# yeyupiaoling/PPASR

Hardware: AMD Instinct MI355X
Metric: audio-seconds/s (RTF^-1) Conformer-streaming fbank, batch32 per GPU, ctc_greedy (higher is better)
Workload: dtype f32; 1 GPU; configs[1]: Conformer streaming (configs/conformer.yml), fbank-80, 32 x 10 s utterances per GPU, V=4233, ctc_greedy, features resident in HBM -> token ids + scores on device; global_batch=32, frames=1000, decoder=ctc_greedy, parallelism=utterance-dp1, pipelined=False, gemm=f32

## Files before the change

### ppasr_amd/csrc/capi.hip

```cpp
#include <cstdlib>

#include "capi_internal.h"

namespace ppasr {
thread_local LaunchProf g_launch_prof;
}

static thread_local std::string g_err;
std::string& ppasr_err_slot() { return g_err; }

static ppasr_status validate_desc(const ppasr_model_desc* desc, ppasr_model_s* m) {
  m->desc = *desc;
  const int F = desc->input_dim;
  if (desc->model_type == PPASR_MODEL_DEEPSPEECH2) {
    if (F > 128 || F < 7) return fail(PPASR_EUNSUPPORTED, "input_dim out of range");
    m->F1 = (F - 1) / 2;
    m->F2 = (m->F1 - 1) / 2;
    if (m->F1 > 40) return fail(PPASR_EUNSUPPORTED, "deepspeech2: input_dim <= 82 ((input_dim - 1) / 2 <= 40)");
    return PPASR_OK;
  }
  if (desc->model_type != PPASR_MODEL_CONFORMER && desc->model_type != PPASR_MODEL_SQUEEZEFORMER &&
      desc->model_type != PPASR_MODEL_EFFICIENT_CONFORMER)
    return fail(PPASR_EUNSUPPORTED, "model_type not built (conformer, efficient_conformer, squeezeformer are)");
  const bool eff = desc->model_type == PPASR_MODEL_EFFICIENT_CONFORMER;
// ... 30 lines not shown
    return fail(PPASR_EINVAL, "PPASR_OPT_SQ_NO_ADAPTIVE_SCALE / PPASR_OPT_SQ_PRE_NORM are Squeezeformer options");
  if (desc->linear_units % 256 != 0 || desc->linear_units <= 0) return fail(PPASR_EUNSUPPORTED, "linear_units % 256 != 0");
  if (!generic && !fused_ks) return fail(PPASR_EUNSUPPORTED, "cnn_module_kernel must be 7, 15 or 31");
  if (generic) {
    const int ks = desc->cnn_module_kernel;
    const bool use_cnn = !(desc->options & PPASR_OPT_NO_CNN);
    if (use_cnn && (ks < 1 || ks > 63 || (!desc->causal && ks % 2 == 0)))
      return fail(PPASR_EINVAL, "cnn_module_kernel: 1..63, odd for the non-causal conv module (convolution.py:38)");
    if ((desc->options & PPASR_OPT_POS_MASK) == 3 || ((desc->options >> PPASR_OPT_ACT_SHIFT) & PPASR_OPT_ACT_MASK) > PPASR_ACT_HARDSHRINK)
      return fail(PPASR_EINVAL, "options: unknown pos_enc_layer_type / activation_type code");
  }
  if (desc->model_type == PPASR_MODEL_SQUEEZEFORMER && desc->cnn_module_kernel == 7)
    return fail(PPASR_EUNSUPPORTED, "squeezeformer: cnn_module_kernel must be 15 or 31");
  if (desc->input_dim > 128 || (desc->input_dim < 7 && desc->input_layer != 1) || desc->input_dim < 1)
    return fail(PPASR_EUNSUPPORTED, "input_dim out of range");
  if (eff) {
    m->desc.stride_layer_mask = (int)smask;
    m->desc.stride_layer_idx = smask ? __builtin_ctz(smask) : -1;
  }
  const int il = desc->input_layer;
  if (il != 0 && il != 1 && il != 6 && il != 8)
    return fail(PPASR_EINVAL, "input_layer: 0 (conv2d), 1 (linear), 6 (conv2d6) or 8 (conv2d8)");
  m->generic = generic;
  m->gen.pos = desc->options & PPASR_OPT_POS_MASK;
  m->gen.post_norm = (desc->options & PPASR_OPT_POST_NORM) != 0;
  m->gen.concat_after = (desc->options & PPASR_OPT_CONCAT_AFTER) != 0;
  m->gen.macaron = !(desc->options & PPASR_OPT_NO_MACARON);
  m->gen.use_cnn = !(desc->options & PPASR_OPT_NO_CNN);
  m->gen.act = (desc->options >> PPASR_OPT_ACT_SHIFT) & PPASR_OPT_ACT_MASK;
  m->gen.sq_pre_norm = (desc->options & PPASR_OPT_SQ_PRE_NORM) != 0;
  if (il != 0 && desc->model_type == PPASR_MODEL_SQUEEZEFORMER)
    return fail(PPASR_EUNSUPPORTED, "squeezeformer: only the conv2d front end is built");
  m->F1 = (F - 1) / 2;
  if (il == 6 && m->F1 < 5) return fail(PPASR_EINVAL, "input_dim too small for this input_layer (conv2d6: >= 11)");
  m->F2 = il == 6 ? (m->F1 - 5) / 3 + 1 : (m->F1 - 1) / 2;
  m->F3 = il == 8 ? (m->F2 - 1) / 2 : 0;
  if (il != 1 && m->F_last() < 1) return fail(PPASR_EINVAL, "input_dim too small for this input_layer");
  return PPASR_OK;
}

extern "C" {

const char* ppasr_last_error(void) { return g_err.c_str(); }
const char* ppasr_version(void) { return "ppasr_hip 0.1 (gfx950, fp32 MFMA)"; }

ppasr_status ppasr_create(const ppasr_model_desc* desc, const ppasr_weight_blob* blobs, int n_blobs, ppasr_handle* out) {
  if (!desc || !blobs || !out) return fail(PPASR_EINVAL, "null argument");
  std::unique_ptr<ppasr_model_s> m(new ppasr_model_s());
  LOAD_TRY(validate_desc(desc, m.get()));
  HIP_TRY(configure_kernels());
  if (desc->model_type != PPASR_MODEL_DEEPSPEECH2) {
    HIP_TRY(configure_generic_kernels());
    HIP_TRY(configure_squeezeformer_kernels());
  }
  const BlobMap sd = blob_map(blobs, n_blobs);
  Loader ld{m.get(), sd, ""};
  switch (desc->model_type) {
    case PPASR_MODEL_DEEPSPEECH2: LOAD_TRY(ds2_create(m.get(), ld)); break;
    case PPASR_MODEL_SQUEEZEFORMER: LOAD_TRY(squeezeformer_create(m.get(), ld)); break;
    default: LOAD_TRY(conformer_create(m.get(), ld));
  }
  HIP_TRY(hipDeviceSynchronize());
  *out = m.release();
  return PPASR_OK;
}

ppasr_status ppasr_destroy(ppasr_handle h) {
  delete h;
  return PPASR_OK;
}

int ppasr_out_frames(ppasr_handle h, int T) {
  if (T < (h ? h->min_frames() : 7)) return 0;
  int tp = h ? h->front_dims(T).Tp : ((T - 1) / 2 - 1) / 2;
  if (h)
    for (int n = __builtin_popcount(eff_stride_mask(h->desc)); n > 0; --n) tp = (tp + 1) / 2;
  return tp;
}

}
WsLayout ws_layout(const ppasr_model_s* m, int B, int T) {
  if (m->generic) {
    WsLayout g{};
    g.total = generic_ws_floats(m, B, T);
    return g;
  }
  const auto fd = m->front_dims(T);
  const size_t T1 = fd.T1, Tp = fd.Tp;
  const size_t M = (size_t)B * Tp;
  auto al = [](size_t n) { return (n + 63) & ~(size_t)63; };
  WsLayout w;
  size_t o = 0;
  const size_t split_rows = m->ffn_split > 1 ? (size_t)m->ffn_split * M
                          : m->ffn_split == 0 ? 0 : std::min((size_t)8 * M, (size_t)256 * kRows);
  w.y1 = o; o += al(std::max((size_t)B * T1 * m->F1 * kD, 4 * split_rows * kD));
  const size_t y2_floats = (size_t)B * (fd.T2 ? fd.T2 : Tp) * m->F2 * kD;
  w.y2 = o; o += al(m->desc.input_layer == 8 ? std::max(y2_floats, split_rows * kD) : y2_floats);
  w.xa = o; o += al(M * kD);
  w.xb = o; o += al(M * kD);
  w.xc = o; o += al(M * kD);
  w.qkv = o; o += al(M * 3 * kD);
  w.ctx = o; o += al(M * kD);
  w.g = o; o += al(M * kD);
  w.rmax = o; o += al(M);
  w.rsum = o; o += al(M);
  w.fa = o; o += al(M);
// ... 463 lines not shown
```

### ppasr_amd/csrc/capi_internal.h

```cpp
#pragma once
#include <hip/hip_runtime.h>

#include <cmath>
#include <cstdio>
#include <cstring>
#include <memory>
#include <string>
#include <unordered_map>
#include <vector>

#include "../../include/ppasr_hip.h"
#include "conformer_kernels.h"
#include "launch.h"
#include "ctc_beam.h"

using namespace ppasr;

#include "squeezeformer_kernels.h"
#include "ds2_kernels.h"
#include "rescore_kernels.h"

std::string& ppasr_err_slot();
inline ppasr_status fail(ppasr_status s, const std::string& msg) {
  ppasr_err_slot() = msg;
// ... 138 lines not shown
  };
  int sub_rate() const { return desc.input_layer == 1 ? 1 : desc.input_layer ? desc.input_layer : 4; }
  int F_last() const { return desc.input_layer == 8 ? F3 : F2; }
  int min_frames() const { return desc.input_layer == 1 ? 1 : desc.input_layer == 6 ? 11 : desc.input_layer == 8 ? 15 : 7; }
  Front front_dims(int T) const {
    if (desc.input_layer == 1) return Front{0, 0, T};
    Front f{(T - 1) / 2, 0, 0};
    if (desc.input_layer == 6) {
      f.Tp = (f.T1 - 5) / 3 + 1;
    } else if (desc.input_layer == 8) {
      f.T2 = (f.T1 - 1) / 2;
      f.Tp = (f.T2 - 1) / 2;
    } else {
      f.Tp = (f.T1 - 1) / 2;
    }
    return f;
  }
  bool generic = false;
  struct GenOpts {
    int pos = 0;
    bool post_norm = false, concat_after = false, macaron = true, use_cnn = true;
    int act = 0;
    bool sq_pre_norm = false;
  } gen;
  struct GenLayerX {
    const f32x4* wcat = nullptr;
    const float* bcat = nullptr;
  };
  std::vector<GenLayerX> gen_x;
  const float* pe_dev = nullptr;
  const float* zero_vec = nullptr;
  const float *lin_ln_g = nullptr, *lin_ln_b = nullptr;
  int lin_kpad = 0;
  FrontW front;
  std::vector<LayerW> layers;
  std::vector<int> layer_ks;
  std::vector<int> layer_group;
  HeadW head;
  std::vector<SqLayerW> sq_layers;
  SqReduceW sq_reduce{};
  const f32x4* sq_wrec = nullptr;
  const float* sq_brec = nullptr;
  const float *preln_g = nullptr, *preln_b = nullptr;
  Ds2W ds2{};
  int ds2_persist_hold = 0, ds2_persist_giveups = 0;
  std::vector<Ds2LayerW> ds2_layers;
  float* taps = nullptr;
  size_t taps_floats = 0;
  float* memory_out = nullptr;
  size_t memory_floats = 0;
  bool sq_final_proj = false;
  bool prof = false;
  int front_fused = -1;
  int ffn_split = -1;
  bool skip_padding = false;
  int gemm_mode = 0;
  std::vector<LayerW> layers_h3;
  const f32x4* conv2_w_h3 = nullptr;
  const f32x4* embed_w_h3 = nullptr;
  const f32x4* head_w_h3 = nullptr;
  std::vector<SqLayerW> sq_layers_h3;
  bool h3_layers() const { return gemm_mode == PPASR_GEMM_F16X3 && !layers_h3.empty(); }
  bool h3_sq_layers() const { return gemm_mode == PPASR_GEMM_F16X3 && !sq_layers_h3.empty(); }
  int gemm_coverage = 0;
  bool gemm_guard = true;
  static constexpr int kGuardN = 5;
  unsigned int* guard_ctr[kGuardN] = {};
  unsigned int* guard_dev = nullptr;
  unsigned int* guard_host = nullptr;
  unsigned int guard_seen[kGuardN] = {};
  long long guard_fallbacks = 0, guard_events = 0;
  int row_block = -1;
  std::vector<int64_t> lens_hint;
  std::vector<hipEvent_t> ev_pool;
  size_t ev_used = 0;
  struct Span { int cls; std::vector<std::pair<hipEvent_t, hipEvent_t>> ev; };
  std::vector<Span> spans;

  ppasr_status upload(const std::vector<float>& v, const float** out) {
    return upload_bytes(v.data(), v.size() * sizeof(float), reinterpret_cast<const void**>(out));
  }
  ppasr_status upload4(const std::vector<float>& v, const f32x4** out) {
    return upload_bytes(v.data(), v.size() * sizeof(float), reinterpret_cast<const void**>(out));
  }
  hipEvent_t next_event() {
    if (ev_used == ev_pool.size()) {
      hipEvent_t e;
      (void)hipEventCreate(&e);
      ev_pool.push_back(e);
    }
    return ev_pool[ev_used++];
  }
  ~ppasr_model_s() {
    for (hipEvent_t e : ev_pool) (void)hipEventDestroy(e);
    if (guard_host) (void)hipHostFree(guard_host);
  }
};


struct ppasr_stream_s {
  ppasr_model_s* m;
  int D;
  int cap;
  int cache_t;
  int cache_r;
  int offset;
// ... 58 lines not shown
```

### ppasr_amd/csrc/conformer_kernels.h

```cpp
#pragma once
#include <hip/hip_runtime.h>
#include <stdint.h>

#include "rowblock.h"

namespace ppasr {

struct LayerW {
  const float *ln_mac_g, *ln_mac_b, *ln_mha_g, *ln_mha_b, *ln_conv_g, *ln_conv_b;
  const float *ln_ff_g, *ln_ff_b, *ln_fin_g, *ln_fin_b, *ln_cm_g, *ln_cm_b;
  float cm_eps;
  const f32x4 *ffm_w1, *ffm_w2, *ff_w1, *ff_w2, *wqkv, *wo, *pw1, *pw2;
  const float *ffm_b1, *ffm_b2, *ff_b1, *ff_b2, *bqkv, *bo, *pw1_b, *pw2_b;
  const float *dw_w;
  const float *dw_b;
  const float *glu_pad;
  const float *pos_u, *pos_v;
  const float *ptab;
  const float *dtab = nullptr;
};

struct FrontW {
  const float *cmvn_mean, *cmvn_istd;
  const float *conv1_w, *conv1_b;
// ... 17 lines not shown
struct SessDesc {
  int sess;
  int cache_t;
  int pos0;
  int offset;
};

struct AttnArgs {
  const float* q;
  int q_stride;
  const float* k;
  int k_stride;
  const float* v;
  int v_stride;
  int T1, T2;
  int pos0;
  const int64_t* lens;
  float* ctx;
  const float *pos_u, *pos_v;
  const float* ptab;
  int pos_stride;
  int mask_mul;
  int q_frames, kv_frames;
  int group;
  const SessDesc* sess;
  long long sess_stride;
  int pad_skip;
  const float* vt = nullptr;
  int vt_stride = 0;
  int dm = 256;
  const float* dtab = nullptr;
  int dtab_len = 0;
};
struct VtOut {
  float* vt = nullptr;
  int stride = 0;
  int k_h3 = 0;
  const float* kpos = nullptr;
  int kpos_stride = 0;
  int Ti = 1;
};

constexpr size_t kLdsExclusive = 82 * 1024;
size_t ragged_lds(size_t lds, const PadSkip& ps, int n_blocks);

bool launch_attention_t(const AttnArgs& a, int B, int H, hipStream_t st);
hipError_t configure_attention_kernels();

void launch_block_table(const PadSkip& ps, int M, int R, int* tab, hipStream_t st);

bool conv2_quad_supported(const FrontW& fw);
bool conv12_supported(const FrontW& fw, int F, int F2);
void launch_conv12(const float* feats, const FrontW& fw, float* y2, int B, int T, int F, int Tp, int F2, hipStream_t st,
                   const PadSkip& ps_frames, int* tile_scratch);
void launch_conv2_quad(const float* y1, const FrontW& fw, float* y2, int B, int T1, int F1, int Tp, int F2, hipStream_t st,
                       const PadSkip& ps_frames, int* tile_scratch);
hipError_t configure_front_fused_kernels();

void launch_out_glu_split_16(const float* ctx, const float* x1, float* x2, float* g, float* xhat, const LayerW& w,
                             const int64_t* lens, int M, int Tp, int mask_mul, hipStream_t st, const PadSkip& ps,
                             float* hist = nullptr, int lo = 0);
void launch_shift_caches(float* kc, float* vc, long long layer_stride, int D, int n_layers, int from_full, int keep_full,
                         int from_half, int keep_half, unsigned long long half_mask, hipStream_t st);
void launch_oproj_ln_16(const float* ctx, const float* x1, float* x2_sink, float* xhat_out, const LayerW& w, int M,
                        hipStream_t st, const PadSkip& ps = PadSkip{});
void launch_pw1_glu_cols_16(const float* x, float* g, const LayerW& w, int M, hipStream_t st, float* hist = nullptr, int lo = 0,
                            const float* hist_scale = nullptr, const float* hist_bias = nullptr, const PadSkip& ps = PadSkip{},
                            const int64_t* lens = nullptr, int Tp = 1, int mask_mul = 1);
bool conv_ffn_16_supported(int ksize, int Tp);
hipError_t configure_conformer_t_kernels();

template <int R>
struct LayerStagesT {
  static hipError_t configure();
  static void ffn_qkv(const float* x_in, float* x1, float* qkv, const LayerW& w, int M, int n_chunks, hipStream_t st,
                      const PadSkip& ps, VtOut vt);
  static void out_glu(const float* ctx, const float* x1, float* x2, float* g, const LayerW& w, const int64_t* lens, int M,
                      int Tp, int mask_mul, hipStream_t st, const PadSkip& ps, float* xhat_out = nullptr,
                      int stop_after_ln = 0);
  static void conv_ffn(const float* g, const float* x2, float* x_out, const LayerW& w, const int64_t* lens, int M, int Tp,
                       int n_chunks, int ksize, int mask_mul, const LayerW* next, float* x1_next, float* qkv_next,
                       hipStream_t st, bool causal, const PadSkip& ps, VtOut vt_next);
};

void launch_posproj(const float* pe, const float* wpos , const float* bpos_or_null, float* ptab,
                    int max_len, hipStream_t st, int d = 256);
void launch_pos_dtab(const float* ptab, const float* pos_u, const float* pos_v, float* dtab, int max_len, hipStream_t st);
void launch_conv1(const float* feats, const FrontW& fw, float* y1, int B, int T, int F, int T1, int F1, hipStream_t st,
                  const PadSkip& ps = PadSkip{}, int channels = 256);
void launch_conv_stage(const float* y_in, const f32x4* w, const float* bias, float* y_out, int B, int T_in, int F_in,
                       int T_out, int F_out, int k, int s, hipStream_t st, const PadSkip& ps_frames = PadSkip{},
                       int channels = 256, int* tile_scratch = nullptr,
                       bool h3 = false,
                       float* part = nullptr, size_t part_floats = 0);
size_t conv_stage_part_floats(int M, int channels = 256);
size_t conv_stage_part_reserve(int M);
void launch_conv2(const float* y1, const FrontW& fw, float* y2, int B, int T1, int F1, int Tp, int F2, hipStream_t st,
                  const PadSkip& ps = PadSkip{}, int* tile_scratch = nullptr, const f32x4* w_h3 = nullptr, float* part = nullptr,
                  size_t part_floats = 0);
void launch_embed(const float* y2, const FrontW& fw, float* x0, int M, int K, float xscale, bool scale_before_bias,
                  hipStream_t st, const PadSkip& ps = PadSkip{}, int k_slices = 1, float* part = nullptr,
                  const f32x4* w_h3 = nullptr);
void launch_dense(const float* a, int lda, const f32x4* w, const float* bias, float* out, int M, int K, int n_cols_padded,
                  int ldc, int n_valid, hipStream_t st, float scale = 1.0f, float* part = nullptr, size_t part_floats = 0);
void launch_ffn_qkv(const float* x_in, float* x1, float* qkv, const LayerW& w, int M, int n_chunks, hipStream_t st,
                    const PadSkip& ps = PadSkip{}, VtOut vt = VtOut{}, bool h3 = false, int rows = 32);
void launch_repack_h3(const f32x4* src, f32x4* dst, int n_tiles, int G, unsigned int* ovf, hipStream_t st);
inline bool conv_ffn_h3_supported(int ksize) { return ksize == 15 || ksize == 7; }
void launch_split_rows_h3(const float* src, float* dst, long long n_rows, unsigned int* ovf, hipStream_t st);
// ... 88 lines not shown
```

### ppasr_amd/csrc/encode_common.h

```cpp
#pragma once

struct RaggedPlan {
  bool skip;
  const int64_t* lens;
  int rc;
  bool rate_changes;
  int mul0;
  int slack(int mul) const { return rate_changes && mul == mul0 ? 2 * (rc + 4) + rc + 8 : rc + 4; }
  PadSkip at(int Tcur, int mul) const {
    PadSkip ps;
    if (skip) {
      ps.lens = lens;
      ps.Tp = Tcur;
      ps.mul = mul;
      ps.slack = slack(mul);
    }
    return ps;
  }
  int attn_pad_skip(const PadSkip& ps) const { return skip ? ps.slack + 1 : 0; }
};

struct BlockTables {
  struct Tab { int Ti, R; int* tab; } tabs[4];
  int n = 0, B;
// ... 5 lines not shown
      : B(B_), off(((size_t)B_ + 2 + 15) / 16 * 16), cap(2 * (((size_t)M + 63) / 64 * 64)), base(reinterpret_cast<int*>(stats)), st(st_) {
    fits = (size_t)B + 2 <= cap / 2;
    on = skip && fits && block_tables_enabled();
  }
  int* tile_tab() const { return fits ? base : nullptr; }
  PadSkip make(PadSkip p, int Tcur, int R) {
    const size_t len = 1 + ((size_t)B * Tcur + R - 1) / R;
    if (!on || n == 4 || off + len > cap) return p;
    int* t = base + off;
    launch_block_table(p, B * Tcur, R, t, st);
    tabs[n++] = Tab{Tcur, R, t};
    off += (len + 15) / 16 * 16;
    p.tab = t;
    return p;
  }
  PadSkip with_table(PadSkip p, int Tcur, int R) {
    for (int k = 0; k < n; ++k)
      if (tabs[k].Ti == Tcur && tabs[k].R == R) {
        p.tab = tabs[k].tab;
        return p;
      }
    return make(p, Tcur, R);
  }
};

struct Taps {
  float* buf;
  size_t cap;
  hipStream_t st;
  size_t off = 0;
  void operator()(const float* src, size_t n_floats) {
    if (buf && off + n_floats <= cap)
      (void)hipMemcpyAsync(buf + off, src, n_floats * sizeof(float), hipMemcpyDeviceToDevice, st);
    off += n_floats;
  }
};

struct NoSpans {
  template <typename Fn>
  void operator()(int, Fn&& fn) const { fn(); }
};

template <typename Spans>
inline void front4_fused(const ppasr_model_s* h, const float* feats, int B, int T, const PadSkip& ps, int* tile_tab,
                         bool scale_before_bias, int embed_slices, const PadSkip& ps_embed, float* y1, float* y2, float* xa,
                         hipStream_t st, Spans&& spans) {
  const auto fd = h->front_dims(T);
  const int F = h->desc.input_dim, T1 = fd.T1, F1 = h->F1, Tp = fd.Tp, F2 = h->F2;
  const bool il4 = h->desc.input_layer == 0;
  const f32x4* conv2_h3 = h->gemm_mode == PPASR_GEMM_F16X3 ? h->conv2_w_h3 : nullptr;
  const bool conv12 = il4 && !conv2_h3 && conv12_enabled(h) && conv12_supported(h->front, F, F2);
  if (!conv12) spans(0, [&] { launch_conv1(feats, h->front, y1, B, T, F, T1, F1, st, ps); });
  spans(1, [&] {
    if (conv12) launch_conv12(feats, h->front, y2, B, T, F, Tp, F2, st, ps, tile_tab);
    else if (il4 && !conv2_h3 && conv2_quad_supported(h->front)) launch_conv2_quad(y1, h->front, y2, B, T1, F1, Tp, F2, st, ps, tile_tab);
    else launch_conv2(y1, h->front, y2, B, T1, F1, Tp, F2, st, ps, tile_tab, il4 ? conv2_h3 : nullptr);
  });
  spans(2, [&] {
    launch_embed(y2, h->front, xa, B * Tp, F2 * kD, sqrtf((float)kD), scale_before_bias, st, ps_embed, embed_slices, y1,
                 conv2_h3 ? h->embed_w_h3 : nullptr);
  });
}

inline ppasr_status memory_out(const ppasr_model_s* h, const float* x, const float* g, const float* b, int M, int D,
                               const PadSkip& ps, hipStream_t st) {
  if (!h->memory_out) return PPASR_OK;
  if ((size_t)M * D > h->memory_floats) return fail(PPASR_ENOSPACE, "memory buffer too small (ppasr_set_memory_out)");
  launch_memory_out(x, g, b, h->memory_out, M, D, ps, st);
  return PPASR_OK;
}

template <typename Spans>
inline ppasr_status fused_head_tail(const ppasr_model_s* h, const float* x, float* probs, float* logits, int32_t* frame_argmax,
                                    float* frame_maxprob, float* ws, const WsLayout& wl, int B, int M, int slices,
                                    const PadSkip& ps, hipStream_t st, Spans&& spans) {
  if (ppasr_status ms = memory_out(h, x, h->head.ln_g, h->head.ln_b, M, kD, ps, st)) return ms;
  float* lg = logits ? logits : probs;
  int32_t* fa = frame_argmax ? frame_argmax : reinterpret_cast<int32_t*>(ws + wl.fa);
  float* fp = frame_maxprob ? frame_maxprob : ws + wl.fp;
  spans(7, [&] {
    const bool head_h3 = h->gemm_mode == PPASR_GEMM_F16X3 && h->head_w_h3;
    HeadW hw = h->head;
    if (head_h3) hw.w = h->head_w_h3;
    launch_ctc_head(x, hw, lg, fa, fp, ws + wl.rmax, ws + wl.rsum, M, st, ps, slices, ws + wl.y1, head_h3);
  });
  if (probs) {
    if (logits) HIP_TRY(hipMemcpyAsync(probs, logits, (size_t)M * h->head.V * sizeof(float), hipMemcpyDeviceToDevice, st));
    launch_softmax_from_stats(probs, ws + wl.rmax, ws + wl.rsum, M, h->head.V, st, ps);
  }
  if (ps.lens) launch_zero_pad_rows(probs, logits, fa, fp, ps.lens, B, ps.Tp, ps.mul, h->head.V, st);
  HIP_TRY(hipGetLastError());
  return PPASR_OK;
}

struct LayerRoute {
  int form;
  int S;
  bool fuse_attn;
  bool h3, h3s;
};
inline bool fuse_rows(const ppasr_model_s* h, int rows) {
  constexpr int fuse_min_blocks = 128;
  return ffn_split_for(h, rows) == 1 && (h->ffn_split == 0 || (rows + kRows - 1) / kRows > fuse_min_blocks);
}
inline LayerRoute layer_route(const ppasr_model_s* h, int B, int Ti, int mul, int slack, bool skip, int layer) {
  const int Mi = B * Ti;
  LayerRoute r;
  const int rows = (!h->taps && conv_ffn_16_supported(h->layer_ks[layer], Ti)) ? row_block_for(h, B, Ti, mul, slack, skip) : 32;
// ... 10 lines not shown
```

### ppasr_amd/csrc/front_fused.hip

```cpp
#include <utility>

#include "conformer_kernels.h"
#include "launch.h"

namespace ppasr {

namespace {
constexpr int kGroupRow[5] = {2, 0, 1, 4, 3};
constexpr int kTapCol[5] = {2, 0, 1, 4, 3};
constexpr int kFactor[5] = {2, 0, 1, 3, 1};
constexpr int quad_slab(int t) { return 4 * kFactor[t / 5] + kFactor[t % 5]; }
constexpr int quad_target(int t) {
  const int g = t / 5, k = t % 5;
  if (g == 0) return k == 0 ? 4 : k <= 2 ? 5 : 4;
  const int a = (g == 1 || g == 2) ? 0 : 2;
  return k == 0 ? (a == 0 ? 5 : 4) : k <= 2 ? a : a + 1;
}
constexpr int quad_fold_src(int t) {
  return t == 1 || t == 5 || t == 21 || t == 23 ? 4 : t == 3 || t == 11 || t == 13 ? 5 : -1;
}
constexpr int quad_fold_mask(int t) {
  return t == 1 ? 0xf : t == 3 ? 0x5 : t == 5 ? 0xa : t == 11 ? 0x2 : t == 13 ? 0x1 : t == 21 ? 0x8 : t == 23 ? 0x4 : 0;
}
constexpr bool quad_fold_clear(int t) { return t == 1 || t == 3 || t == 5 || t == 13 || t == 23; }
static_assert(quad_target(0) == 4 && quad_target(2) == 5 && quad_target(10) == 5 && quad_target(12) == 0 &&
                  quad_target(14) == 1 && quad_target(20) == 4 && quad_target(22) == 2 && quad_target(24) == 3,
              "chunk targets");

template <typename Fn, int... I>
__device__ __forceinline__ void static_for(std::integer_sequence<int, I...>, Fn&& fn) {
  (fn(std::integral_constant<int, I>{}), ...);
}

__host__ __device__ inline int quad_xs_stride(int F, int Q) { return F > 8 * Q + 3 ? F : 8 * Q + 3; }
}

template <bool FROM_Y1>
__device__ __forceinline__ void conv2_quad_body(const float* __restrict__ src, const FrontW& fw, float* __restrict__ out,
                                                int T, int F, int Tp, int F2, int M, int m0, const PadSkip& ps,
                                                const int* __restrict__ tile_tab) {
  constexpr int BP = 32, KC = 128, LD = KC + 4, G = KC / 8, NL = 2, N_CHUNKS = 25;
  constexpr int SLOT = BP * LD;
  const int P = (Tp + 1) >> 1;
  const int Q = (F2 + 1) >> 1;
  int r0 = m0 + blockIdx.x * BP, Mlim = M;
  if (tile_tab) {
    const int t = blockIdx.x, nb = tile_tab[0];
    const int* pre = tile_tab + 1;
    if (t >= pre[nb]) return;
    int lo = 0, hi = nb;
    while (hi - lo > 1) {
      const int mid = (lo + hi) >> 1;
      if (pre[mid] <= t) lo = mid;
      else hi = mid;
    }
    const int S = ps.Tp * ps.unit;
    r0 = lo * S + (t - pre[lo]) * BP;
    Mlim = min(M, (lo + 1) * S);
  } else if (pad_block_skippable(ps, r0, BP, M)) {
    return;
  }
  extern __shared__ __attribute__((aligned(16))) float smem[];
  float* const slot0 = smem;
  float* const slot1 = smem + SLOT;
  f32x4* const y2s = reinterpret_cast<f32x4*>(smem + 2 * SLOT);
  float* const w1s = smem + 2 * SLOT + 5 * NL * 4 * kThreads;
  float* const xs = w1s + 10 * 256;
  const int tid = threadIdx.x, lane = lane_id(), wave = wave_id();
  constexpr int tile_stride = 2 * 16 * G * 64;
  const f32x4* wbase = fw.conv2_wp + (size_t)wave * tile_stride;
  auto seg = [&](int h, int slab) { return wbase + (size_t)(16 * h + slab) * G * 64; };
  BRing<1> ring;
  ring_prime(ring, seg(0, quad_slab(0)), 0);
  const int c4 = tid & 31, rbase = tid >> 5;
  const int bp0 = r0 / Q;
  const int FX = quad_xs_stride(F, Q);
  uint32_t pb = 0;
  int yrow[FROM_Y1 ? NL : 1], yp4[FROM_Y1 ? NL : 1], yq4[FROM_Y1 ? NL : 1];
  if constexpr (!FROM_Y1) {
    for (int idx = tid; idx < 10 * 256; idx += kThreads) w1s[idx] = idx < 9 * 256 ? fw.conv1_w[idx] : fw.conv1_b[idx - 9 * 256];
    const int nbp = (min(r0 + BP, Mlim) - 1) / Q - bp0 + 1;
    for (int idx = tid; idx < nbp * 11 * FX; idx += kThreads) {
      const int fr_row = idx / FX, f = idx - fr_row * FX;
      const int bpl = fr_row / 11, fr = fr_row - 11 * bpl;
      const int bp = bp0 + bpl, b = bp / P, p = bp - b * P;
      const int t = min(8 * p + fr, T - 1);
      xs[idx] = f < F ? (src[((size_t)b * T + t) * F + f] - fw.cmvn_mean[f]) * fw.cmvn_istd[f] : 0.f;
    }
#pragma unroll
    for (int i = 0; i < NL; ++i) {
      const int m = r0 + rbase + 16 * i;
      const int bp = m / Q, q = m - bp * Q;
      const uint32_t v = m < Mlim ? (uint32_t)((bp - bp0) * 11 * FX + 8 * q) : 0xffffu;
      pb |= v << (16 * i);
    }
  } else {
#pragma unroll
    for (int i = 0; i < NL; ++i) {
      const int m = r0 + rbase + 16 * i;
      const int bp = m / Q, q = m - bp * Q, b = bp / P, p = bp - b * P;
      yrow[i] = b * T + 4 * p;
      yp4[i] = 4 * p;
      yq4[i] = m < Mlim ? 4 * q : -1;
    }
  }
  auto pbase = [&](int i) { return (int)((pb >> (16 * i)) & 0xffffu); };
  const int lds_off0 = rbase * LD + 4 * c4;
  float xv[9];
  f32x4 wv[3], bv, ya, yv;
  auto y1_step = [&](int i, int h, int r, int c, int step) {
    const int cc = h * 128 + 4 * c4;
    if constexpr (!FROM_Y1) {
      if (step == 0) {
        const int o = pbase(i);
        const float* p = xs + (o == 0xffff ? 0 : o) + 2 * r * FX + 2 * c;
#pragma unroll
        for (int ii = 0; ii < 3; ++ii)
#pragma unroll
          for (int jj = 0; jj < 3; ++jj) xv[ii * 3 + jj] = p[ii * FX + jj];
        ya = f32x4{0.f, 0.f, 0.f, 0.f};
      } else {
#pragma unroll
        for (int j = 3 * (step - 1); j < 3 * step; ++j)
#pragma unroll
          for (int e = 0; e < 4; ++e) ya[e] = fmaf(wv[j % 3][e], xv[j], ya[e]);
        if (step == 3) {
          ya += bv;
#pragma unroll
          for (int e = 0; e < 4; ++e) ya[e] = pbase(i) != 0xffff ? fmaxf(ya[e], 0.f) : 0.f;
        }
      }
      if (step < 3) {
#pragma unroll
        for (int j = 0; j < 3; ++j) wv[j] = *reinterpret_cast<const f32x4*>(w1s + (3 * step + j) * 256 + cc);
        if (step == 2) bv = *reinterpret_cast<const f32x4*>(w1s + 9 * 256 + cc);
      }
    } else {
      if (step == 0) {
        yv = f32x4{0.f, 0.f, 0.f, 0.f};
        if (yq4[i] >= 0 && yp4[i] + r < T && yq4[i] + c < F)
          yv = *reinterpret_cast<const f32x4*>(src + ((size_t)(yrow[i] + r) * F + yq4[i] + c) * 256 + cc);
      } else if (step == 3) {
        ya = yv;
      }
    }
  };
  auto put = [&](float* buf, int i, const f32x4& v) { *reinterpret_cast<f32x4*>(buf + lds_off0 + i * 16 * LD) = v; };
  auto y2row = [&](int c, int i) -> f32x4& { return y2s[(c * NL + i) * kThreads + tid]; };
  f32x4 z2[NL];
  auto build = [&](auto nc, int g, int h, float* buf) {
    constexpr int n = decltype(nc)::value, grp = n / 5, k = n % 5, r = kGroupRow[grp], c = kTapCol[k];
    const int i = g >> 2, step = g & 3;
    y1_step(i, h, r, c, step);
    if (step != 3) return;
    f32x4 v = ya;
    if constexpr (grp == 0) y2row(c, i) = ya;
    if constexpr (grp == 1 || grp == 3) v = ya - y2row(c, i);
    if constexpr (k == 0) {
      z2[i] = v;
      put(buf, i, v);
    } else if constexpr (k == 1 || k == 3) {
      put(buf, i, v - z2[i]);
    } else {
      put(buf, i, v);
    }
  };
  f32x16 acc[6][1][1];
#pragma unroll
  for (int a = 0; a < 6; ++a) acc_zero(acc[a]);
  auto fold = [&](auto tc, int g) {
    constexpr int t = decltype(tc)::value, fs = quad_fold_src(t), mask = quad_fold_mask(t);
    if constexpr (fs >= 0) {
      const int j = g - 4 * NL;
      int seen = 0;
#pragma unroll
      for (int o = 0; o < 4; ++o) {
        if (!((mask >> o) & 1)) continue;
        if (seen++ == j) {
#pragma unroll
          for (int e = 0; e < 16; ++e) asm volatile("v_add_f32 %0, %0, %1" : "+v"(acc[o][0][0][e]) : "v"(acc[fs][0][0][e]));
        }
      }
      if (quad_fold_clear(t) && j == 4) acc_zero(acc[fs]);
    }
  };
  __syncthreads();
#pragma unroll
  for (int g = 0; g < 4 * NL; ++g) {
    build(std::integral_constant<int, 0>{}, g, 0, slot0);
    __builtin_amdgcn_sched_barrier(0);
  }
  __syncthreads();
  for (int h = 0; h < 2; ++h) {
    asm volatile("" : "+s"(wbase));
    if constexpr (!FROM_Y1) {
      asm volatile("" : "+v"(pb));
    } else {
#pragma unroll
      for (int i = 0; i < NL; ++i) asm volatile("" : "+v"(yrow[i]), "+v"(yp4[i]), "+v"(yq4[i]));
    }
    static_for(std::make_integer_sequence<int, N_CHUNKS>{}, [&](auto tc) {
      constexpr int t = decltype(tc)::value;
      float* const cur = ((t + h) & 1) ? slot1 : slot0;
      float* const nxb = ((t + h) & 1) ? slot0 : slot1;
      const f32x4* nseg = t + 1 < N_CHUNKS ? seg(h, quad_slab(t + 1)) : (h == 0 ? seg(1, quad_slab(0)) : nullptr);
      auto side = [&](int g) {
        if (g < 4 * NL) {
          if constexpr (t + 1 < N_CHUNKS) build(std::integral_constant<int, t + 1>{}, g, h, nxb);
          else if (h == 0) build(std::integral_constant<int, 0>{}, g, 1, nxb);
        } else {
          fold(tc, g);
        }
      };
      rb_gemm<1, 1, G, kPF, decltype(side)>(cur, LD, seg(h, quad_slab(t)), 0, nseg, 0, ring, acc[quad_target(t)], side);
      __syncthreads();
    });
  }
  const int col = wave * 32 + (lane & 31);
  const float b2 = fw.conv2_b[col];
#pragma unroll
  for (int r = 0; r < 16; ++r) {
    const int m = r0 + acc_row(r, lane);
    if (m >= Mlim) continue;
    const int bp = m / Q, q = m - bp * Q, b = bp / P, t0 = 2 * (bp - b * P), f0 = 2 * q;
    float* o = out + ((size_t)(b * Tp + t0) * F2 + f0) * 256 + col;
    const bool f1 = f0 + 1 < F2, t1 = t0 + 1 < Tp;
    o[0] = fmaxf(acc[0][0][0][r] + b2, 0.f);
    if (f1) o[256] = fmaxf(acc[1][0][0][r] + b2, 0.f);
    if (t1) o[(size_t)F2 * 256] = fmaxf(acc[2][0][0][r] + b2, 0.f);
    if (t1 && f1) o[(size_t)F2 * 256 + 256] = fmaxf(acc[3][0][0][r] + b2, 0.f);
  }
}

__global__ __launch_bounds__(kThreads) void k_conv12(const float* __restrict__ feats, FrontW fw, float* __restrict__ out,
                                                     int T, int F, int Tp, int F2, int M, int m0, PadSkip ps,
                                                     const int* __restrict__ tile_tab) {
  conv2_quad_body<false>(feats, fw, out, T, F, Tp, F2, M, m0, ps, tile_tab);
}
__global__ __launch_bounds__(kThreads) void k_conv2_pair(const float* __restrict__ y1, FrontW fw, float* __restrict__ out,
                                                         int T1, int F1, int Tp, int F2, int M, int m0, PadSkip ps,
                                                         const int* __restrict__ tile_tab) {
  conv2_quad_body<true>(y1, fw, out, T1, F1, Tp, F2, M, m0, ps, tile_tab);
}

static int quad_tile_pairs(int Q) { return 31 / Q + 2; }
static size_t quad_lds(bool fused, int F, int F2) {
  const int Q = (F2 + 1) / 2;
  return ((size_t)2 * 32 * 132 + (size_t)5 * 2 * 4 * 512 + (fused ? (size_t)10 * 256 + (size_t)quad_tile_pairs(Q) * 11 * quad_xs_stride(F, Q) : 0)) *
         sizeof(float);
}
bool conv2_quad_supported(const FrontW& fw) { return fw.conv2_wp && fw.conv2_k == 3 && fw.conv2_s == 2; }
bool conv12_supported(const FrontW& fw, int F, int F2) {
  const int Q = (F2 + 1) / 2;
  return conv2_quad_supported(fw) && F2 >= 1 && quad_lds(true, F, F2) <= 160 * 1024 &&
         (size_t)quad_tile_pairs(Q) * 11 * quad_xs_stride(F, Q) < 0xffff;
}

void launch_tile_prefix(const PadSkip& ps, int B, int BM, int* tab, hipStream_t st);

static void launch_quad(bool fused, const float* src, const FrontW& fw, float* y2, int B, int T, int F, int Tp, int F2,
                        hipStream_t st, const PadSkip& ps_frames, int* tile_scratch) {
  const int P = (Tp + 1) / 2, Q = (F2 + 1) / 2;
  PadSkip ps = ps_frames;
  ps.Tp = P;
  ps.mul = 2 * ps_frames.mul;
  ps.slack = (ps_frames.slack + 1) / 2;
  ps.unit = Q;
  const int M = B * P * Q;
  const int* no_tab = nullptr;
#define QUAD(GRID, TAB)                                                                                                  \
  do {                                                                                                                 \
    if (fused)                                                                                                         \
      PPASR_LAUNCH(k_conv12, dim3(GRID), dim3(kThreads), quad_lds(true, F, F2), st, src, fw, y2, T, F, Tp, F2, M, 0, ps, \
                   TAB);                                                                                               \
    else                                                                                                               \
      PPASR_LAUNCH(k_conv2_pair, dim3(GRID), dim3(kThreads), quad_lds(false, F, F2), st, src, fw, y2, T, F, Tp, F2, M, 0, \
                   ps, TAB);                                                                                           \
  } while (0)
  if (ps.lens && tile_scratch) {
    launch_tile_prefix(ps, B, 32, tile_scratch, st);
    QUAD(B * ((P * Q + 31) / 32), (const int*)tile_scratch);
    return;
  }
  QUAD((M + 31) / 32, no_tab);
#undef QUAD
}

void launch_conv12(const float* feats, const FrontW& fw, float* y2, int B, int T, int F, int Tp, int F2, hipStream_t st,
                   const PadSkip& ps_frames, int* tile_scratch) {
  launch_quad(true, feats, fw, y2, B, T, F, Tp, F2, st, ps_frames, tile_scratch);
}
void launch_conv2_quad(const float* y1, const FrontW& fw, float* y2, int B, int T1, int F1, int Tp, int F2, hipStream_t st,
                       const PadSkip& ps_frames, int* tile_scratch) {
  launch_quad(false, y1, fw, y2, B, T1, F1, Tp, F2, st, ps_frames, tile_scratch);
}

hipError_t configure_front_fused_kernels() {
  hipError_t e;
#define SET_LDS(fn)                                                                                              \
  e = hipFuncSetAttribute(reinterpret_cast<const void*>(fn), hipFuncAttributeMaxDynamicSharedMemorySize, 160 * 1024); \
  if (e != hipSuccess) return e;
  SET_LDS(k_conv12);
  SET_LDS(k_conv2_pair);
#undef SET_LDS
  return hipSuccess;
}

}
```

Before: 58460 audio-s/s.

## Make fused conv1+conv2 front kernel persistent with prefetch of next tile's input patch

Converts the fused conv12 subsampling kernel into a persistent grid-stride loop capped at the CU count, so each block processes several tiles. While the final GEMM chunk of the current tile runs, the next tile's CMVN-normalized input patch is loaded into registers and committed to LDS, overlapping global loads with compute. This cuts block launch and weight-setup overhead, but adds register pressure and fewer resident blocks, which may hurt latency hiding. It also adds an env override for the grid size and timestamp probes.

```diff
diff --git a/ppasr_amd/csrc/capi.hip b/ppasr_amd/csrc/capi.hip
--- a/ppasr_amd/csrc/capi.hip
+++ b/ppasr_amd/csrc/capi.hip
@@ -106,6 +106,15 @@
   if (desc->model_type != PPASR_MODEL_DEEPSPEECH2) {
     HIP_TRY(configure_generic_kernels());
     HIP_TRY(configure_squeezeformer_kernels());
+  }
+  {
+    int dev = 0, cus = 0;
+    HIP_TRY(hipGetDevice(&dev));
+    HIP_TRY(hipDeviceGetAttribute(&cus, hipDeviceAttributeMultiprocessorCount, dev));
+    const char* e = getenv("PPASR_CONV12_GRID");
+    const int cap = e ? atoi(e) : 0;
+    m->front_grid = cap > 0 ? cap : std::max(cus, 1);
+    m->front_grid_twin = cap > 0 ? cap : 0;
   }
   const BlobMap sd = blob_map(blobs, n_blobs);
   Loader ld{m.get(), sd, ""};
diff --git a/ppasr_amd/csrc/capi_internal.h b/ppasr_amd/csrc/capi_internal.h
--- a/ppasr_amd/csrc/capi_internal.h
+++ b/ppasr_amd/csrc/capi_internal.h
@@ -214,6 +214,7 @@
   bool sq_final_proj = false;
   bool prof = false;
   int front_fused = -1;
+  int front_grid = 0, front_grid_twin = 0;
   int ffn_split = -1;
   bool skip_padding = false;
   int gemm_mode = 0;
diff --git a/ppasr_amd/csrc/conformer_kernels.h b/ppasr_amd/csrc/conformer_kernels.h
--- a/ppasr_amd/csrc/conformer_kernels.h
+++ b/ppasr_amd/csrc/conformer_kernels.h
@@ -93,9 +93,9 @@
 bool conv2_quad_supported(const FrontW& fw);
 bool conv12_supported(const FrontW& fw, int F, int F2);
 void launch_conv12(const float* feats, const FrontW& fw, float* y2, int B, int T, int F, int Tp, int F2, hipStream_t st,
-                   const PadSkip& ps_frames, int* tile_scratch);
+                   const PadSkip& ps_frames, int* tile_scratch, int grid_cap);
 void launch_conv2_quad(const float* y1, const FrontW& fw, float* y2, int B, int T1, int F1, int Tp, int F2, hipStream_t st,
-                       const PadSkip& ps_frames, int* tile_scratch);
+                       const PadSkip& ps_frames, int* tile_scratch, int grid_cap);
 hipError_t configure_front_fused_kernels();
 
 void launch_out_glu_split_16(const float* ctx, const float* x1, float* x2, float* g, float* xhat, const LayerW& w,
diff --git a/ppasr_amd/csrc/encode_common.h b/ppasr_amd/csrc/encode_common.h
--- a/ppasr_amd/csrc/encode_common.h
+++ b/ppasr_amd/csrc/encode_common.h
@@ -81,8 +81,8 @@
   const bool conv12 = il4 && !conv2_h3 && conv12_enabled(h) && conv12_supported(h->front, F, F2);
   if (!conv12) spans(0, [&] { launch_conv1(feats, h->front, y1, B, T, F, T1, F1, st, ps); });
   spans(1, [&] {
-    if (conv12) launch_conv12(feats, h->front, y2, B, T, F, Tp, F2, st, ps, tile_tab);
-    else if (il4 && !conv2_h3 && conv2_quad_supported(h->front)) launch_conv2_quad(y1, h->front, y2, B, T1, F1, Tp, F2, st, ps, tile_tab);
+    if (conv12) launch_conv12(feats, h->front, y2, B, T, F, Tp, F2, st, ps, tile_tab, h->front_grid);
+    else if (il4 && !conv2_h3 && conv2_quad_supported(h->front)) launch_conv2_quad(y1, h->front, y2, B, T1, F1, Tp, F2, st, ps, tile_tab, h->front_grid_twin);
     else launch_conv2(y1, h->front, y2, B, T1, F1, Tp, F2, st, ps, tile_tab, il4 ? conv2_h3 : nullptr);
   });
   spans(2, [&] {
diff --git a/ppasr_amd/csrc/front_fused.hip b/ppasr_amd/csrc/front_fused.hip
--- a/ppasr_amd/csrc/front_fused.hip
+++ b/ppasr_amd/csrc/front_fused.hip
@@ -1,9 +1,18 @@
+#include <algorithm>
+#include <climits>
 #include <utility>
 
 #include "conformer_kernels.h"
 #include "launch.h"
 
 namespace ppasr {
+#ifdef PPASR_PHASE_TS
+}
+extern "C" __attribute__((visibility("default"))) int ppasr_debug_read_phase_ts_fused(long long* out) {
+  return (int)hipMemcpyFromSymbol(out, HIP_SYMBOL(ppasr::g_phase_ts), sizeof(long long) * 128);
+}
+namespace ppasr {
+#endif
 
 namespace {
 constexpr int kGroupRow[5] = {2, 0, 1, 4, 3};
@@ -33,6 +42,7 @@
 }
 
 __host__ __device__ inline int quad_xs_stride(int F, int Q) { return F > 8 * Q + 3 ? F : 8 * Q + 3; }
+__host__ __device__ inline int quad_tile_pairs(int Q) { return 31 / Q + 2; }
 }
 
 template <bool FROM_Y1>
@@ -43,23 +53,34 @@
   constexpr int SLOT = BP * LD;
   const int P = (Tp + 1) >> 1;
   const int Q = (F2 + 1) >> 1;
-  int r0 = m0 + blockIdx.x * BP, Mlim = M;
-  if (tile_tab) {
-    const int t = blockIdx.x, nb = tile_tab[0];
-    const int* pre = tile_tab + 1;
-    if (t >= pre[nb]) return;
-    int lo = 0, hi = nb;
-    while (hi - lo > 1) {
-      const int mid = (lo + hi) >> 1;
-      if (pre[mid] <= t) lo = mid;
-      else hi = mid;
-    }
-    const int S = ps.Tp * ps.unit;
-    r0 = lo * S + (t - pre[lo]) * BP;
-    Mlim = min(M, (lo + 1) * S);
-  } else if (pad_block_skippable(ps, r0, BP, M)) {
-    return;
-  }
+  const int n_tiles = tile_tab ? (tile_tab + 1)[tile_tab[0]] : (M - m0 + BP - 1) / BP;
+  auto locate = [&](int t, int& r0_, int& Mlim_) {
+    for (; t < n_tiles; t += gridDim.x) {
+      if (tile_tab) {
+        const int nb = tile_tab[0];
+        const int* pre = tile_tab + 1;
+        int lo = 0, hi = nb;
+        while (hi - lo > 1) {
+          const int mid = (lo + hi) >> 1;
+          if (pre[mid] <= t) lo = mid;
+          else hi = mid;
+        }
+        const int S = ps.Tp * ps.unit;
+        r0_ = lo * S + (t - pre[lo]) * BP;
+        Mlim_ = min(M, (lo + 1) * S);
+        return t;
+      }
+      r0_ = m0 + t * BP;
+      Mlim_ = M;
+      if (!pad_block_skippable(ps, r0_, BP, M)) return t;
+    }
+    return -1;
+  };
+  int r0 = 0, Mlim = 0;
+  int tile = locate(blockIdx.x, r0, Mlim);
+  if (tile < 0) return;
+  [[maybe_unused]] int ts_k = 0;
+  PPASR_TS(0);
   extern __shared__ __attribute__((aligned(16))) float smem[];
   float* const slot0 = smem;
   float* const slot1 = smem + SLOT;
@@ -67,43 +88,100 @@
   float* const w1s = smem + 2 * SLOT + 5 * NL * 4 * kThreads;
   float* const xs = w1s + 10 * 256;
   const int tid = threadIdx.x, lane = lane_id(), wave = wave_id();
+  auto opaque = [](int v) {
+    asm volatile("" : "+v"(v));
+    return v;
+  };
   constexpr int tile_stride = 2 * 16 * G * 64;
   const f32x4* wbase = fw.conv2_wp + (size_t)wave * tile_stride;
   auto seg = [&](int h, int slab) { return wbase + (size_t)(16 * h + slab) * G * 64; };
   BRing<1> ring;
   ring_prime(ring, seg(0, quad_slab(0)), 0);
   const int c4 = tid & 31, rbase = tid >> 5;
-  const int bp0 = r0 / Q;
   const int FX = quad_xs_stride(F, Q);
+  auto patch_rows = [&](int r0_, int Mlim_) { return ((min(r0_ + BP, Mlim_) - 1) / Q - r0_ / Q + 1) * 11; };
+  auto patch_src = [&](int r0_, int rr) {
+    const int bpl = rr / 11, fr = rr - 11 * bpl;
+    const int bp = r0_ / Q + bpl, b = bp / P, p = bp - b * P;
+    const int t = min(8 * p + fr, T - 1);
+    return src + ((size_t)b * T + t) * F;
+  };
+  auto patch_fill = [&](int r0_, int Mlim_) {
+    const int nr = patch_rows(r0_, Mlim_), tl = opaque(tid);
+    for (int rr = tl >> 5; rr < nr; rr += 16) {
+      const float* row = patch_src(r0_, rr);
+      for (int f = tl & 31; f < FX; f += 32) xs[rr * FX + f] = f < F ? (row[f] - fw.cmvn_mean[f]) * fw.cmvn_istd[f] : 0.f;
+    }
+  };
+  constexpr int PFJ = 4, PFK = 3;
+  const bool pf_ok = !FROM_Y1 && quad_tile_pairs(Q) * 11 <= 16 * PFJ && FX <= 32 * PFK;
+  float pf[PFJ][PFK], pf_m[PFK], pf_s[PFK];
+  auto patch_request = [&](int r0_, int Mlim_) {
+    const int nr = patch_rows(r0_, Mlim_), tl = opaque(tid);
+#pragma unroll
+    for (int k = 0; k < PFK; ++k) {
+      const int f = (tl & 31) + 32 * k;
+      pf_m[k] = f < F ? fw.cmvn_mean[f] : 0.f;
+      pf_s[k] = f < F ? fw.cmvn_istd[f] : 0.f;
+    }
+#pragma unroll
+    for (int j = 0; j < PFJ; ++j) {
+      const int rr = (tl >> 5) + 16 * j;
+      const float* row = patch_src(r0_, rr < nr ? rr : 0);
+#pragma unroll
+      for (int k = 0; k < PFK; ++k) {
+        const int f = (tl & 31) + 32 * k;
+        pf[j][k] = rr < nr && f < F ? row[f] : 0.f;
+      }
+    }
+  };
+  auto patch_commit = [&](int r0_, int Mlim_) {
+    const int nr = patch_rows(r0_, Mlim_), tl = opaque(tid);
+#pragma unroll
+    for (int j = 0; j < PFJ; ++j) {
+      const int rr = (tl >> 5) + 16 * j;
+#pragma unroll
+      for (int k = 0; k < PFK; ++k) {
+        const int f = (tl & 31) + 32 * k;
+        if (rr < nr && f < FX) xs[rr * FX + f] = f < F ? (pf[j][k] - pf_m[k]) * pf_s[k] : 0.f;
+      }
+    }
+  };
   uint32_t pb = 0;
   int yrow[FROM_Y1 ? NL : 1], yp4[FROM_Y1 ? NL : 1], yq4[FROM_Y1 ? NL : 1];
+  auto row_state = [&](int r0_, int Mlim_) {
+    const int bp0 = r0_ / Q;
+    const int rbase = opaque(tid) >> 5;
+    if constexpr (!FROM_Y1) {
+      pb = 0;
+#pragma unroll
+      for (int i = 0; i < NL; ++i) {
+        const int m = r0_ + rbase + 16 * i;
+        const int bp = m / Q, q = m - bp * Q;
+        const uint32_t v = m < Mlim_ ? (uint32_t)((bp - bp0) * 11 * FX + 8 * q) : 0u;
+        pb |= v << (16 * i);
+      }
+    } else {
+#pragma unroll
+      for (int i = 0; i < NL; ++i) {
+        const int m = r0_ + rbase + 16 * i;
+        const int bp = m / Q, q = m - bp * Q, b = bp / P, p = bp - b * P;
+        yrow[i] = b * T + 4 * p;
+        yp4[i] = 4 * p;
+        yq4[i] = m < Mlim_ ? 4 * q : -1;
+      }
+    }
+  };
   if constexpr (!FROM_Y1) {
     for (int idx = tid; idx < 10 * 256; idx += kThreads) w1s[idx] = idx < 9 * 256 ? fw.conv1_w[idx] : fw.conv1_b[idx - 9 * 256];
-    const int nbp = (min(r0 + BP, Mlim) - 1) / Q - bp0 + 1;
-    for (int idx = tid; idx < nbp * 11 * FX; idx += kThreads) {
-      const int fr_row = idx / FX, f = idx - fr_row * FX;
-      const int bpl = fr_row / 11, fr = fr_row - 11 * bpl;
-      const int bp = bp0 + bpl, b = bp / P, p = bp - b * P;
-      const int t = min(8 * p + fr, T - 1);
-      xs[idx] = f < F ? (src[((size_t)b * T + t) * F + f] - fw.cmvn_mean[f]) * fw.cmvn_istd[f] : 0.f;
-    }
-#pragma unroll
-    for (int i = 0; i < NL; ++i) {
-      const int m = r0 + rbase + 16 * i;
-      const int bp = m / Q, q = m - bp * Q;
-      const uint32_t v = m < Mlim ? (uint32_t)((bp - bp0) * 11 * FX + 8 * q) : 0xffffu;
-      pb |= v << (16 * i);
-    }
-  } else {
-#pragma unroll
-    for (int i = 0; i < NL; ++i) {
-      const int m = r0 + rbase + 16 * i;
-      const int bp = m / Q, q = m - bp * Q, b = bp / P, p = bp - b * P;
-      yrow[i] = b * T + 4 * p;
-      yp4[i] = 4 * p;
-      yq4[i] = m < Mlim ? 4 * q : -1;
+    if (pf_ok) {
+      patch_request(r0, Mlim);
+      patch_commit(r0, Mlim);
+    } else {
+      patch_fill(r0, Mlim);
     }
   }
+  row_state(r0, Mlim);
   auto pbase = [&](int i) { return (int)((pb >> (16 * i)) & 0xffffu); };
   const int lds_off0 = rbase * LD + 4 * c4;
   float xv[9];
@@ -112,8 +190,7 @@
     const int cc = h * 128 + 4 * c4;
     if constexpr (!FROM_Y1) {
       if (step == 0) {
-        const int o = pbase(i);
-        const float* p = xs + (o == 0xffff ? 0 : o) + 2 * r * FX + 2 * c;
+        const float* p = xs + pbase(i) + 2 * r * FX + 2 * c;
 #pragma unroll
         for (int ii = 0; ii < 3; ++ii)
 #pragma unroll
@@ -127,7 +204,7 @@
         if (step == 3) {
           ya += bv;
 #pragma unroll
-          for (int e = 0; e < 4; ++e) ya[e] = pbase(i) != 0xffff ? fmaxf(ya[e], 0.f) : 0.f;
+          for (int e = 0; e < 4; ++e) ya[e] = fmaxf(ya[e], 0.f);
         }
       }
       if (step < 3) {
@@ -185,50 +262,99 @@
     }
   };
   __syncthreads();
-#pragma unroll
-  for (int g = 0; g < 4 * NL; ++g) {
-    build(std::integral_constant<int, 0>{}, g, 0, slot0);
-    __builtin_amdgcn_sched_barrier(0);
-  }
-  __syncthreads();
-  for (int h = 0; h < 2; ++h) {
-    asm volatile("" : "+s"(wbase));
+  PPASR_TS(1);
+  for (;;) {
+#pragma unroll
+    for (int g = 0; g < 4 * NL; ++g) {
+      build(std::integral_constant<int, 0>{}, g, 0, slot0);
+      __builtin_amdgcn_sched_barrier(0);
+    }
+    __syncthreads();
+    PPASR_TS(8 * (ts_k & 7) + 2);
+    int r0n = 0, Mlimn = 0;
+    const int tile_n = locate(tile + gridDim.x, r0n, Mlimn);
+    for (int h = 0; h < 2; ++h) {
+      asm volatile("" : "+s"(wbase));
+      if constexpr (!FROM_Y1) {
+        asm volatile("" : "+v"(pb));
+      } else {
+#pragma unroll
+        for (int i = 0; i < NL; ++i) asm volatile("" : "+v"(yrow[i]), "+v"(yp4[i]), "+v"(yq4[i]));
+      }
+      static_for(std::make_integer_sequence<int, N_CHUNKS>{}, [&](auto tc) {
+        constexpr int t = decltype(tc)::value;
+        float* const cur = ((t + h) & 1) ? slot1 : slot0;
+        float* const nxb = ((t + h) & 1) ? slot0 : slot1;
+        const f32x4* nseg = t + 1 < N_CHUNKS ? seg(h, quad_slab(t + 1)) : seg(h ^ 1, quad_slab(0));
+        auto gemm = [&](auto side) {
+          rb_gemm<1, 1, G, kPF, decltype(side)>(cur, LD, seg(h, quad_slab(t)), 0, nseg, 0, ring, acc[quad_target(t)], side);
+        };
+        if constexpr (t + 1 < N_CHUNKS) {
+          gemm([&](int g) {
+            if (g < 4 * NL) build(std::integral_constant<int, t + 1>{}, g, h, nxb);
+            else fold(tc, g);
+          });
+        } else if (h == 0) {
+          gemm([&](int g) {
+            if (g < 4 * NL) build(std::integral_constant<int, 0>{}, g, 1, nxb);
+          });
+        } else if (pf_ok && tile_n >= 0) {
+          gemm([&](int g) {
+            if (g == 0) patch_request(r0n, Mlimn);
+            else if (g == G - 4) patch_commit(r0n, Mlimn);
+          });
+        } else {
+          gemm(NoSide());
+        }
+        __syncthreads();
+      });
+    }
+    PPASR_TS(8 * (ts_k & 7) + 3);
+    {
+      const int le = opaque(lane), col = wave * 32 + (le & 31);
+      const float b2 = fw.conv2_b[col];
+      int m = r0 + 4 * (le >> 5);
+      const int bp = m / Q, b = bp / P;
+      int q = m - bp * Q, p = bp - b * P;
+      float* o = out + ((size_t)(b * Tp + 2 * p) * F2 + 2 * q) * 256 + col;
+      const ptrdiff_t dq = (ptrdiff_t)(2 * F2 - 2 * Q) * 256;
+      const ptrdiff_t dp = (ptrdiff_t)(Tp - 2 * P) * F2 * 256;
+      auto step = [&] {
+        ++m, ++q, o += 512;
+        if (q == Q) {
+          q = 0, ++p, o += dq;
+          if (p == P) p = 0, o += dp;
+        }
+      };
+#pragma unroll
+      for (int r = 0; r < 16; ++r) {
+        if (m < Mlim) {
+          const bool f1 = 2 * q + 1 < F2, t1 = 2 * p + 1 < Tp;
+          o[0] = fmaxf(acc[0][0][0][r] + b2, 0.f);
+          if (f1) o[256] = fmaxf(acc[1][0][0][r] + b2, 0.f);
+          if (t1) o[(size_t)F2 * 256] = fmaxf(acc[2][0][0][r] + b2, 0.f);
+          if (t1 && f1) o[(size_t)F2 * 256 + 256] = fmaxf(acc[3][0][0][r] + b2, 0.f);
+        }
+        if (r < 15) {
+          step();
+          if ((r & 3) == 3) step(), step(), step(), step();
+        }
+      }
+    }
+    PPASR_TS(8 * (ts_k & 7) + 4);
+    if (tile_n < 0) break;
+    tile = tile_n, r0 = r0n, Mlim = Mlimn;
+    ++ts_k;
+    PPASR_TS(8 * (ts_k & 7));
     if constexpr (!FROM_Y1) {
-      asm volatile("" : "+v"(pb));
-    } else {
-#pragma unroll
-      for (int i = 0; i < NL; ++i) asm volatile("" : "+v"(yrow[i]), "+v"(yp4[i]), "+v"(yq4[i]));
-    }
-    static_for(std::make_integer_sequence<int, N_CHUNKS>{}, [&](auto tc) {
-      constexpr int t = decltype(tc)::value;
-      float* const cur = ((t + h) & 1) ? slot1 : slot0;
-      float* const nxb = ((t + h) & 1) ? slot0 : slot1;
-      const f32x4* nseg = t + 1 < N_CHUNKS ? seg(h, quad_slab(t + 1)) : (h == 0 ? seg(1, quad_slab(0)) : nullptr);
-      auto side = [&](int g) {
-        if (g < 4 * NL) {
-          if constexpr (t + 1 < N_CHUNKS) build(std::integral_constant<int, t + 1>{}, g, h, nxb);
-          else if (h == 0) build(std::integral_constant<int, 0>{}, g, 1, nxb);
-        } else {
-          fold(tc, g);
-        }
-      };
-      rb_gemm<1, 1, G, kPF, decltype(side)>(cur, LD, seg(h, quad_slab(t)), 0, nseg, 0, ring, acc[quad_target(t)], side);
-      __syncthreads();
-    });
-  }
-  const int col = wave * 32 + (lane & 31);
-  const float b2 = fw.conv2_b[col];
-#pragma unroll
-  for (int r = 0; r < 16; ++r) {
-    const int m = r0 + acc_row(r, lane);
-    if (m >= Mlim) continue;
-    const int bp = m / Q, q = m - bp * Q, b = bp / P, t0 = 2 * (bp - b * P), f0 = 2 * q;
-    float* o = out + ((size_t)(b * Tp + t0) * F2 + f0) * 256 + col;
-    const bool f1 = f0 + 1 < F2, t1 = t0 + 1 < Tp;
-    o[0] = fmaxf(acc[0][0][0][r] + b2, 0.f);
-    if (f1) o[256] = fmaxf(acc[1][0][0][r] + b2, 0.f);
-    if (t1) o[(size_t)F2 * 256] = fmaxf(acc[2][0][0][r] + b2, 0.f);
-    if (t1 && f1) o[(size_t)F2 * 256 + 256] = fmaxf(acc[3][0][0][r] + b2, 0.f);
+      if (!pf_ok) {
+        patch_fill(r0, Mlim);
+        __syncthreads();
+      }
+    }
+    row_state(r0, Mlim);
+    acc_zero(acc[0]), acc_zero(acc[1]), acc_zero(acc[2]), acc_zero(acc[3]);
+    PPASR_TS(8 * (ts_k & 7) + 1);
   }
 }
 
@@ -243,7 +369,6 @@
   conv2_quad_body<true>(y1, fw, out, T1, F1, Tp, F2, M, m0, ps, tile_tab);
 }
 
-static int quad_tile_pairs(int Q) { return 31 / Q + 2; }
 static size_t quad_lds(bool fused, int F, int F2) {
   const int Q = (F2 + 1) / 2;
   return ((size_t)2 * 32 * 132 + (size_t)5 * 2 * 4 * 512 + (fused ? (size_t)10 * 256 + (size_t)quad_tile_pairs(Q) * 11 * quad_xs_stride(F, Q) : 0)) *
@@ -259,7 +384,7 @@
 void launch_tile_prefix(const PadSkip& ps, int B, int BM, int* tab, hipStream_t st);
 
 static void launch_quad(bool fused, const float* src, const FrontW& fw, float* y2, int B, int T, int F, int Tp, int F2,
-                        hipStream_t st, const PadSkip& ps_frames, int* tile_scratch) {
+                        hipStream_t st, const PadSkip& ps_frames, int* tile_scratch, int grid_cap) {
   const int P = (Tp + 1) / 2, Q = (F2 + 1) / 2;
   PadSkip ps = ps_frames;
   ps.Tp = P;
@@ -277,22 +402,23 @@
       PPASR_LAUNCH(k_conv2_pair, dim3(GRID), dim3(kThreads), quad_lds(false, F, F2), st, src, fw, y2, T, F, Tp, F2, M, 0, \
                    ps, TAB);                                                                                           \
   } while (0)
+  const int cap = grid_cap > 0 ? grid_cap : INT_MAX;
   if (ps.lens && tile_scratch) {
     launch_tile_prefix(ps, B, 32, tile_scratch, st);
-    QUAD(B * ((P * Q + 31) / 32), (const int*)tile_scratch);
+    QUAD(std::min(B * ((P * Q + 31) / 32), cap), (const int*)tile_scratch);
     return;
   }
-  QUAD((M + 31) / 32, no_tab);
+  QUAD(std::min((M + 31) / 32, cap), no_tab);
 #undef QUAD
 }
 
 void launch_conv12(const float* feats, const FrontW& fw, float* y2, int B, int T, int F, int Tp, int F2, hipStream_t st,
-                   const PadSkip& ps_frames, int* tile_scratch) {
-  launch_quad(true, feats, fw, y2, B, T, F, Tp, F2, st, ps_frames, tile_scratch);
+                   const PadSkip& ps_frames, int* tile_scratch, int grid_cap) {
+  launch_quad(true, feats, fw, y2, B, T, F, Tp, F2, st, ps_frames, tile_scratch, grid_cap);
 }
 void launch_conv2_quad(const float* y1, const FrontW& fw, float* y2, int B, int T1, int F1, int Tp, int F2, hipStream_t st,
-                       const PadSkip& ps_frames, int* tile_scratch) {
-  launch_quad(false, y1, fw, y2, B, T1, F1, Tp, F2, st, ps_frames, tile_scratch);
+                       const PadSkip& ps_frames, int* tile_scratch, int grid_cap) {
+  launch_quad(false, y1, fw, y2, B, T1, F1, Tp, F2, st, ps_frames, tile_scratch, grid_cap);
 }
 
 hipError_t configure_front_fused_kernels() {
```

Result: no change. 58760 audio-s/s (median of 6 runs) (+0.5%).
